# zhengfei0908/SBA-GAN

Hardware: AMD Instinct MI355X
Metric: images/sec (G+D step) at 256px (higher is better)
Workload: dtype bf16; 1 GPU; bird_style.yml 3-stage G+D step (64..256px), B=20 per GPU, G_NET variant=model, image_encoder=inception, text_encoder=RNN_ENCODER in the step; global_batch=20, parallelism=dp1, launch=replayer, losses_finite=True

## Files before the change

### sba-gan_amd/csrc/wgrad.hip

```cpp
#include "common.h"
#include "conv_common.h"

namespace {

struct FastDiv {
    uint64_t magic;
    uint32_t d;
};
static inline FastDiv make_fastdiv(uint32_t d, int64_t max_n) {
    FastDiv f;
    f.d = d;
    f.magic = (max_n < (1 << 21) && d > 0) ? (((uint64_t)1 << 42) + d - 1) / d : 0;
    return f;
}
__device__ __forceinline__ uint32_t fdiv(uint32_t n, const FastDiv& f) {
    return f.magic ? (uint32_t)(((uint64_t)n * f.magic) >> 42) : n / f.d;
}

__device__ __forceinline__ void zero_acc(f32x16_t (&acc)[2][2]) {
#pragma unroll
    for (int i = 0; i < 2; ++i)
#pragma unroll
        for (int j = 0; j < 2; ++j)
#pragma unroll
            for (int r = 0; r < 16; ++r) acc[i][j][r] = 0.f;
}
template <int N> __device__ __forceinline__ void zero_acc(f32x16_t (&acc)[N][2][2]) {
#pragma unroll
    for (int s = 0; s < N; ++s) zero_acc(acc[s]);
}

__device__ __forceinline__ void pixel_decode(const int m, const int sub, const int ow, const FastDiv& dsub, const FastDiv& dow,
                                             int& n, int& oy, int& ox) {
    n = (int)fdiv(m, dsub);
    const int rem = m - n * sub;
    oy = (int)fdiv(rem, dow);
    ox = rem - oy * ow;
}

__device__ __forceinline__ bool x_gather(const sba_conv_geom& g, const int IHL, const int IWL, const int n, const int oy, const int ox,
                                         const int ty, const int tx, int64_t& pix) {
    int iy = oy * g.sy + ty, ix = ox * g.sx + tx;
    const bool ok = (iy >= 0) & (iy < IHL) & (ix >= 0) & (ix < IWL);
    if (g.ups) { iy >>= 1; ix >>= 1; }
    pix = (int64_t)(n * g.IH + iy) * g.IW + ix;
    return ok;
}
__device__ __forceinline__ int64_t dy_pixel(const sba_conv_geom& g, const int n, const int oy, const int ox) {
    return (int64_t)(n * g.OH + oy * g.osy + g.ooy) * g.OW + ox * g.osx + g.oox;
}

__device__ __forceinline__ void dw_emit(float* p, const float v, const int mode) {
    if (mode == 1) atomicAdd(p, v);
    else if (mode == 2) *p = v;
    else *p += v;
}
template <bool OWNER>
__device__ __forceinline__ void store_tile(const f32x16_t (&acc)[2][2], float* dwz, const sba_conv_geom& g, const int co0,
                                           const int ci0, const int tap, const int mode, const int lane) {
    const int col_l = lane & 31, rsel = 4 * (lane >> 5);
#pragma unroll
    for (int i = 0; i < 2; ++i)
#pragma unroll
        for (int j = 0; j < 2; ++j)
#pragma unroll
            for (int r = 0; r < 16; ++r) {
                const int co = co0 + i * 32 + (r & 3) + 8 * (r >> 2) + rsel;
                const int ci = ci0 + j * 32 + col_l;
                if (co < g.Cout && ci < g.Cin) {
                    float* p = dwz + ((int64_t)co * g.ntaps + tap) * g.Cin + ci;
                    if (OWNER) dw_emit(p, acc[i][j][r], mode);
                    else if (mode == 2) *p = acc[i][j][r];
                    else atomicAdd(p, acc[i][j][r]);
                }
            }
}

template <typename T> struct WgFrag;

template <> struct WgFrag<bf16_t> {
    static constexpr int ROWS = 64 * 2 + 64;
    static __device__ __forceinline__ bf16x8_t load(const unsigned char* slice, int c32, int lane) {
        const int g16 = lane >> 4, i16 = lane & 15;
        const int cbase = c32 + 16 * (g16 & 1), kbase = 8 * (g16 >> 1);
        const int q = i16 >> 2, p = i16 & 3;
        const unsigned char* a0 = slice + (kbase + q) * ROWS + (cbase + 4 * p) * 2;
        typedef __attribute__((address_space(3))) s16x4_t* lptr;
        s16x4_t lo = __builtin_amdgcn_ds_read_tr16_b64_v4i16((lptr)(a0));
        s16x4_t hi = __builtin_amdgcn_ds_read_tr16_b64_v4i16((lptr)(a0 + 4 * ROWS));
        bf16x8_t r;
        r[0] = lo[0]; r[1] = lo[1]; r[2] = lo[2]; r[3] = lo[3];
        r[4] = hi[0]; r[5] = hi[1]; r[6] = hi[2]; r[7] = hi[3];
        return r;
    }
    static __device__ __forceinline__ void mma(const unsigned char* sa, const unsigned char* sb, int lane,
                                               f32x16_t (&acc)[2][2]) {
        bf16x8_t a[2], b[2];
        a[0] = load(sa, 0, lane); a[1] = load(sa, 32, lane);
        b[0] = load(sb, 0, lane); b[1] = load(sb, 32, lane);
#pragma unroll
        for (int i = 0; i < 2; ++i)
#pragma unroll
            for (int j = 0; j < 2; ++j)
                acc[i][j] = __builtin_amdgcn_mfma_f32_32x32x16_bf16(a[i], b[j], acc[i][j], 0, 0, 0);
    }
};

template <> struct WgFrag<float> {
    static constexpr int ROWS = 64 * 4 + 64;
    static __device__ __forceinline__ void mma(const unsigned char* sa, const unsigned char* sb, int lane,
                                               f32x16_t (&acc)[2][2]) {
        const int r = lane & 31, h = lane >> 5;
#pragma unroll
        for (int kk = 0; kk < 8; ++kk) {
            float a[2], b[2];
#pragma unroll
            for (int i = 0; i < 2; ++i) {
                a[i] = *reinterpret_cast<const float*>(sa + (2 * kk + h) * ROWS + (i * 32 + r) * 4);
                b[i] = *reinterpret_cast<const float*>(sb + (2 * kk + h) * ROWS + (i * 32 + r) * 4);
            }
#pragma unroll
            for (int i = 0; i < 2; ++i)
#pragma unroll
                for (int j = 0; j < 2; ++j)
                    acc[i][j] = __builtin_amdgcn_mfma_f32_32x32x2f32(a[i], b[j], acc[i][j], 0, 0, 0);
        }
    }
};

template <typename T>
__global__ __launch_bounds__(256) void wgrad_kernel(const T* __restrict__ x, const T* __restrict__ dy,
                                                    float* __restrict__ dw, const sba_conv_geom g,
                                                    const int M, const int chunks_per_split,
                                                    const int mode, const FastDiv dsub, const FastDiv dow,
                                                    const int64_t zstride) {
    constexpr int ROWS = WgFrag<T>::ROWS;
    constexpr int CH = 16 / (int)sizeof(T);
    constexpr int CPR = 64 / CH;
    constexpr int LPT = 16 * CPR / 64;
    constexpr int SLICE = 16 * ROWS;
    static_assert(4 * 2 * SLICE >= 64 * 64 * 4, "reduction buffer fits in the staging area");
    __shared__ __attribute__((aligned(16))) unsigned char lds[4 * 2 * SLICE];

    const int tid = threadIdx.x, lane = tid & 63, wid = tid >> 6;
    const int co0 = blockIdx.x * 64;
    const int ci_tiles = (g.Cin + 63) / 64;
    const int tap = blockIdx.y / ci_tiles, ci0 = (blockIdx.y - tap * ci_tiles) * 64;
    int ty = 0, tx = 0;
#pragma unroll
    for (int t = 0; t < SBA_MAX_TAPS; ++t)
        if (t == tap) { ty = g.ty[t]; tx = g.tx[t]; }
    const int IHL = g.ups ? 2 * g.IH : g.IH, IWL = g.ups ? 2 * g.IW : g.IW;
    const int sub = g.OHs * g.OWs;

// ... 568 lines not shown
    for (int kw = 0; kw < 3; ++kw)
        store_tile<false>(acc[kw], dw + (int64_t)blockIdx.z * zstride, g, co0, ci0, kh * 3 + kw, mode, lane);
}

enum WgradFamily { WG_ROW_DMA = 0, WG_SMALL_DMA = 1, WG_SMALL = 2, WG_ROWS = 3, WG_GENERIC = 4 };

struct WgradPlan {
    int family;
    int v[4];
    dim3 grid;
    int block, lds;
    int per_split;
    int mode;
    int npart;
    int wclog;
};

static int pixel_splits(int target_wgs, int wgs, int chunks, int min_chunks, int* per_split) {
    int sp = cdiv(target_wgs, wgs);
    if (sp > chunks / min_chunks) sp = chunks / min_chunks > 0 ? chunks / min_chunks : 1;
    *per_split = cdiv(chunks, sp);
    return cdiv(chunks, *per_split);
}

static bool wgrad_plan(int dtype, const sba_conv_geom* g, int ksplit, bool det_on, WgradPlan* p) {
    if (!geom_ok(g, dtype)) return false;
    if (g->Cin % 8 != 0 || g->Cout % 8 != 0) return false;
    if (g->x_cstride || g->x_coff || g->y_cstride || g->y_coff || g->ntaps > 16) return false;
    const int M = g->N * g->OHs * g->OWs;
    if (ksplit < 1) ksplit = 1;
    const int fw = g->first_write ? 2 : 0;
    const int co_tiles = cdiv(g->Cout, 64), items = cdiv(g->Cin, 64) * g->ntaps;
    const bool dma_ok = dtype == SBA_BF16 && (int64_t)g->N * g->OH * g->OW * g->Cout * 2 < (1ll << 32);
    auto fill = [&](int family, int v0, int v1, int v2, int v3, dim3 grid, int block, int lds, int per_split, int unsplit_mode) {
        *p = WgradPlan{family, {v0, v1, v2, v3}, grid, block, lds, per_split, 0, 0, 0};
        const int nz = (int)grid.z;
        p->npart = det_on && (nz > 1 || family == WG_ROWS) ? nz : 0;
        p->mode = p->npart ? 2 : (nz > 1 ? 1 : unsplit_mode);
        return grid.y <= 65535 && grid.z <= 65535;
    };
    {
        const int kwn = g->ntaps == 16 ? 4 : (g->ntaps == 9 ? 3 : 0), sxy = g->sx;
        bool ok = dma_ok && kwn && g->sy == sxy && (!g->ups || kwn == 3) && g->osy == 1 && g->osx == 1 && g->ooy == 0 &&
                  g->oox == 0 && g->OHs == g->OH && g->OWs == g->OW && g->Cin % 64 == 0 && g->Cout % 64 == 0 &&
                  g->OW >= 4 && (g->OW & (g->OW - 1)) == 0 && !(g->OW == 4 && (g->ups || g->OH != 4)) && M % 32 == 0 &&
                  ((g->OH * g->OW) % 32 == 0 || g->OW == 4);
        ok = ok && ((kwn == 4 && sxy == 2) || (kwn == 3 && sxy == 1));
        for (int t = 0; t < g->ntaps && ok; ++t)
            ok = g->ty[t] == g->ty[(t / kwn) * kwn] && g->tx[t] == g->tx[(t / kwn) * kwn] + (t % kwn);
        if (ok) {
            const int wc = g->OW < 32 ? g->OW : 32;
            int wclog = 0;
            while ((1 << wclog) < wc) ++wclog;
            const int wgs = co_tiles * kwn * (g->Cin / 64);
            constexpr int ROW_WGS = 512;
            int cps32;
            const int sp = pixel_splits(wgs <= 8 ? (ROW_WGS * 3) / 4 : ROW_WGS, wgs, M / 32, 12, &cps32);
            const int xb = kwn == 4 ? 10 : (g->OW == 4 ? 6 : 5);
            const int stage = kwn == 4 ? WgRowCfg<4, 10>::STAGE : (g->OW == 4 ? WgRowCfg<3, 6>::STAGE : WgRowCfg<3, 5>::STAGE);
            if (fill(WG_ROW_DMA, kwn, sxy, xb, 4, dim3(co_tiles, kwn * (g->Cin / 64), sp), 64 * kwn, 4 * stage, cps32, fw)) {
                p->wclog = wclog;
                return true;
            }
        }
    }
    constexpr int SMALL_M = 12000;
    if (M <= SMALL_M && co_tiles * items >= 256) {
        const int wgs = co_tiles * cdiv(items, 4);
        constexpr int SMALL_WGS = 768, SMALL_MINC = 24;
        const int target = wgs >= SMALL_WGS / 2 ? wgs : SMALL_WGS;
        int cps;
        const int split = pixel_splits(target, wgs, cdiv(M, 16), SMALL_MINC, &cps);
        const dim3 grid(co_tiles, cdiv(items, 4), split);
        if (grid.y > 65535 || grid.z > 65535) return false;
        constexpr int DMA_WGS = 512;
        if (fw == 2 && wgs > DMA_WGS && g->Cout % 128 == 0 && dma_ok) {
            fill(WG_SMALL_DMA, 2, 3, 0, 0, dim3(co_tiles / 2, cdiv(items, 4), 1), 256, 3 * 6 * 32 * 128, cdiv(M, 32), fw);
            return true;
        }
        if (wgs <= DMA_WGS && dma_ok) {
            int cps32;
            const int sp = pixel_splits(target, wgs, cdiv(M, 32), SMALL_MINC / 2, &cps32);
            return fill(WG_SMALL_DMA, 1, 4, 0, 0, dim3(co_tiles, cdiv(items, 4), sp), 256, 4 * 5 * 32 * 128, cps32, fw);
        }
        return fill(WG_SMALL, dtype, 0, 0, 0, grid, 256, 0, cps, fw);
    }
    constexpr int ROWS_M = 131072;
    bool rows_ok = g->ntaps == 9 && g->sy == 1 && g->sx == 1 && g->osy == 1 && g->osx == 1 && g->ooy == 0 &&
                   g->oox == 0 && g->OHs == g->OH && g->OWs == g->OW && g->OW % 64 == 0 && M >= ROWS_M;
    for (int t = 0; t < 9 && rows_ok; ++t) rows_ok = g->ty[t] == t / 3 - 1 && g->tx[t] == t % 3 - 1;
    if (rows_ok) {
        const int ci_t = cdiv(g->Cin, 64);
        int spw;
        const int nz = pixel_splits(256, co_tiles * ci_t, g->N * g->OH * (g->OW / 64), 16, &spw);
        return fill(WG_ROWS, dtype, 0, 0, 0, dim3(co_tiles, ci_t, nz), 192, 0, spw, 1);
    }
    if (dma_ok) {
        constexpr int GEN_WGS = 512;
        int cps32;
        const int sp = pixel_splits(GEN_WGS, co_tiles * cdiv(items, 4), cdiv(M, 32), 12, &cps32);
        if (fill(WG_SMALL_DMA, 1, 4, 0, 0, dim3(co_tiles, cdiv(items, 4), sp), 256, 4 * 5 * 32 * 128, cps32, fw)) return true;
    }
    const int total_chunks = cdiv(M, 64);
    if (ksplit > total_chunks) ksplit = total_chunks;
    const int cps = cdiv(total_chunks, ksplit);
    return fill(WG_GENERIC, dtype, 0, 0, 0, dim3(co_tiles, items, cdiv(total_chunks, cps)), 256, 0, cps, 0);
}

template <auto Kernel, typename... Args>
static void launch_dyn_lds(const WgradPlan& p, hipStream_t st, Args... args) {
    static bool once = false;
    if (!once) { (void)hipFuncSetAttribute((const void*)Kernel, hipFuncAttributeMaxDynamicSharedMemorySize, p.lds); once = true; }
    SBA_LAUNCH(Kernel, p.grid, dim3(p.block), p.lds, st, args...);
}

static int wgrad_launch(const WgradPlan& p, int dtype, const void* x, const void* dy, float* dw, const sba_conv_geom* g,
                        hipStream_t st) {
    const int M = g->N * g->OHs * g->OWs;
    const FastDiv dsub = make_fastdiv((uint32_t)(g->OHs * g->OWs), (int64_t)M + 64);
    const FastDiv dow = make_fastdiv((uint32_t)g->OWs, (int64_t)M + 64);
    const int64_t dwn = (int64_t)g->Cout * g->ntaps * g->Cin;
    float* part = nullptr;
    if (p.npart) { part = sba_det_alloc((int64_t)p.npart * dwn); if (!part) return SBA_E_ARG; }
    float* dwa = part ? part : dw;
    const int64_t zs = part ? dwn : 0;
    const bf16_t* xh = (const bf16_t*)x;
    const bf16_t* dyh = (const bf16_t*)dy;
    switch (p.family) {
    case WG_ROW_DMA:
        if (p.v[0] == 4) launch_dyn_lds<wgrad_row_dma_kernel<4, 2, 10, 4>>(p, st, xh, dyh, dwa, *g, M, p.per_split, p.mode, dsub, dow, zs, p.wclog);
        else if (p.v[2] == 6) launch_dyn_lds<wgrad_row_dma_kernel<3, 1, 6, 4>>(p, st, xh, dyh, dwa, *g, M, p.per_split, p.mode, dsub, dow, zs, p.wclog);
        else launch_dyn_lds<wgrad_row_dma_kernel<3, 1, 5, 4>>(p, st, xh, dyh, dwa, *g, M, p.per_split, p.mode, dsub, dow, zs, p.wclog);
        break;
    case WG_SMALL_DMA:
        if (p.v[0] == 2) launch_dyn_lds<wgrad_small_dma_kernel<2, 3>>(p, st, xh, dyh, dwa, *g, M, p.per_split, p.mode, dsub, dow, zs);
        else launch_dyn_lds<wgrad_small_dma_kernel<1, 4>>(p, st, xh, dyh, dwa, *g, M, p.per_split, p.mode, dsub, dow, zs);
        break;
    case WG_SMALL:
        SBA_DISPATCH(dtype, SBA_LAUNCH((wgrad_small_kernel<T>), p.grid, dim3(p.block), 0, st, (const T*)x, (const T*)dy, dwa, *g, M,
                                       p.per_split, p.mode, dsub, dow, zs));
        break;
    case WG_ROWS:
        SBA_DISPATCH(dtype, SBA_LAUNCH((wgrad_rows_kernel<T>), p.grid, dim3(p.block), 0, st, (const T*)x, (const T*)dy, dwa, *g,
                                       g->N * g->OH * (g->OW / 64), p.per_split, p.mode, zs));
        break;
    default:
        SBA_DISPATCH(dtype, SBA_LAUNCH((wgrad_kernel<T>), p.grid, dim3(p.block), 0, st, (const T*)x, (const T*)dy, dwa, *g, M,
                                       p.per_split, p.mode, dsub, dow, zs));
    }
    if (part) sba_det_fold(part, 1, p.npart, dwn, dw, 0, g->first_write ? 1 : 0, st);
    return SBA_CHECK_LAUNCH();
}

}

extern "C" int sba_conv_wgrad_plan(int dtype, const sba_conv_geom* g, int ksplit, int det, int* plan) {
    WgradPlan p;
    if (!plan || !wgrad_plan(dtype, g, ksplit, det != 0, &p)) return SBA_E_ARG;
    const int out[SBA_WGRAD_PLAN_INTS] = {p.family, p.v[0], p.v[1], p.v[2], p.v[3], (int)p.grid.x, (int)p.grid.y, (int)p.grid.z,
                                          p.block, p.lds, p.per_split, p.mode, p.npart, p.wclog};
    for (int i = 0; i < SBA_WGRAD_PLAN_INTS; ++i) plan[i] = out[i];
    return SBA_OK;
}

extern "C" int sba_conv_wgrad(int dtype, const void* x, const void* dy, float* dw, const sba_conv_geom* g,
                              int ksplit, void* stream) {
    WgradPlan p;
    if (!x || !dy || !dw || !wgrad_plan(dtype, g, ksplit, sba_det_on(), &p)) return SBA_E_ARG;
    return wgrad_launch(p, dtype, x, dy, dw, g, (hipStream_t)stream);
}
```

### sba-gan_amd/sbagan/_lib.py

```python
import ctypes
import os

import torch
from ctypes import POINTER, byref, c_float, c_int, c_int64, c_uint64, c_void_p

from .abi import CONSTANTS, DECLS, STRUCTS

_HERE = os.path.dirname(os.path.abspath(__file__))
LIB_PATH = os.environ.get('SBA_LIB_PATH') or os.path.join(os.path.dirname(_HERE), 'csrc', 'libsbagan_hip.so')

SBA_F32, SBA_BF16, SBA_BF16_YH = (CONSTANTS['SBA_' + k] for k in ('F32', 'BF16', 'BF16_YH'))
ACT_NONE, ACT_GLU, ACT_LRELU, ACT_RELU = (CONSTANTS['SBA_ACT_' + k] for k in ('NONE', 'GLU', 'LRELU', 'RELU'))
MAX_TAPS, IGEMM_TILES, WGRAD_PLAN_INTS, GROUP_MAX = (
    CONSTANTS['SBA_' + k] for k in ('MAX_TAPS', 'IGEMM_TILES', 'WGRAD_PLAN_INTS', 'GROUP_MAX'))
WGRAD_FAMILIES = ('row_dma', 'small_dma', 'small', 'rows', 'generic')
ConvGeom, ConvGroupItem = STRUCTS['sba_conv_geom'], STRUCTS['sba_conv_group_item']

if not os.path.exists(LIB_PATH):
    raise ImportError('libsbagan_hip.so not built: run `python __graft_entry__.py` or '
                      '`make -C sba-gan_amd/csrc` (expected %s)' % LIB_PATH)
lib = ctypes.CDLL(LIB_PATH)

P, I, F, L, U = c_void_p, c_int, c_float, c_int64, c_uint64
G = POINTER(ConvGeom)

SIGNATURES = {}
for _name, _decl in DECLS.items():
    _fn = getattr(lib, _name)
    _fn.argtypes = _args = [_ctype for _, _, _ctype in _decl.params]
    _fn.restype = _decl.restype
    if _decl.restype is c_int:
        SIGNATURES[_name] = _args

_ERR = {CONSTANTS['SBA_E_ARG']: 'SBA_E_ARG (unsupported shape/alignment/enum)',
        CONSTANTS['SBA_E_LAUNCH']: 'SBA_E_LAUNCH (HIP launch failed)',
        CONSTANTS['SBA_E_UNSUPPORTED']: 'SBA_E_UNSUPPORTED (graph node kind the replayer cannot re-issue)'}


AUDIT_HOOK = None


def call(name, *args):
    if AUDIT_HOOK is not None:
        AUDIT_HOOK(name, args)
    rc = getattr(lib, name)(*args)
    if rc != 0:
        raise RuntimeError('%s failed: %s' % (name, _ERR.get(rc, rc)))


def wgrad_plan(dtype, g, ksplit, det=None):
    plan = (c_int * WGRAD_PLAN_INTS)()
    det = lib.sba_get_deterministic() if det is None else int(det)
    call('sba_conv_wgrad_plan', dtype, byref(g), ksplit, det, plan)
    return list(plan)


def wgrad_plan_name(plan):
    fam, nargs = WGRAD_FAMILIES[plan[0]], (4, 2, 0, 0, 0)[plan[0]]
    args = ','.join(str(v) for v in plan[1:1 + nargs]) if nargs else ('f32', 'bf16')[plan[1]]
    return '%s<%s> x%d' % (fam, args, plan[7])


def version():
    return lib.sba_version().decode()
```

### sba-gan_amd/sbagan/abi.py

```python
import os
import re
from collections import namedtuple
from ctypes import (POINTER, Structure, c_char_p, c_double, c_float, c_int, c_int8, c_int32, c_int64, c_uint64,
                    c_void_p)

HEADER = os.path.join(os.path.dirname(os.path.dirname(os.path.dirname(os.path.abspath(__file__)))),
                      'include', 'sbagan_hip.h')

TYPES = {'int': c_int, 'int64_t': c_int64, 'uint64_t': c_uint64, 'float': c_float, 'double': c_double,
         'int*': POINTER(c_int), 'void**': POINTER(c_void_p)}
FIELD_TYPES = dict(TYPES, int32_t=c_int32, int8_t=c_int8)
RETURNS = {'int': c_int, 'int64_t': c_int64, 'const char*': c_char_p}
HOST_STRUCTS = ('sba_conv_geom', 'sba_conv_group_item')

Decl = namedtuple('Decl', 'ret restype params')


def _squeeze(ctext):
    return re.sub(r'\s*\*', '*', ' '.join(ctext.split()))


def _ctype(ctext, types, structs, host_structs, where):
    base = re.sub(r'\bconst\b|\s', '', ctext)
    if base in types:
        return types[base]
    if base.endswith('*') and base[:-1] in host_structs:
        if base[:-1] not in structs:
            raise ValueError('%s: %s is used before it is declared' % (where, base[:-1]))
        return POINTER(structs[base[:-1]])
    if re.fullmatch(r'\w+\*+', base):
        return c_void_p
    raise ValueError('%s: unknown type %r' % (where, ctext))


def parse(text, host_structs=HOST_STRUCTS):
    text = re.sub(r'/\*.*?\*/|//[^\n]*', ' ', text, flags=re.S)
    constants, structs, decls = {}, {}, {}

    def new(name):
        if name in constants or name in structs or name in decls:
            raise ValueError('%s is declared twice' % name)
        return name

    for m in re.finditer(r'^[ \t]*#[ \t]*define[ \t]+(SBA_\w+)(.*)$', text, flags=re.M):
        value = re.fullmatch(r'\s+\(?(-?\d+)\)?\s*', m.group(2))
        if not value:
            raise ValueError('#define %s: not an integer: %r' % (m.group(1), m.group(2).strip()))
        constants[new(m.group(1))] = int(value.group(1))
    text = re.sub(r'^[ \t]*#.*$', '', text, flags=re.M)

    def struct(m):
        name, fields = m.group(1), []
        if m.group(3) != name:
            raise ValueError('typedef struct %s: named %s' % (name, m.group(3)))
        for stmt in filter(None, (s.strip() for s in m.group(2).split(';'))):
            f = re.fullmatch(r'(.*?)(\w+(?:\[\w+\])?(?:\s*,\s*\w+(?:\[\w+\])?)*)', stmt, flags=re.S)
            if not f:
                raise ValueError('struct %s: cannot read %r' % (name, stmt))
            ctype = _ctype(f.group(1), FIELD_TYPES, structs, host_structs, 'struct %s: %r' % (name, stmt))
            for field, bound in re.findall(r'(\w+)(?:\[(\w+)\])?', f.group(2)):
                if bound and not bound.isdigit() and bound not in constants:
                    raise ValueError('struct %s: %s[%s]: unknown bound' % (name, field, bound))
                fields.append((field, ctype * int(constants.get(bound, bound)) if bound else ctype))
        structs[new(name)] = type(name, (Structure,), {'_fields_': fields})
        return ''
    text = re.sub(r'typedef\s+struct\s+(\w+)\s*\{(.*?)\}\s*(\w+)\s*;', struct, text, flags=re.S)

    text = re.sub(r'extern\s+"C"\s*\{|\}', '', text)
    for stmt in filter(None, (' '.join(s.split()) for s in text.split(';'))):
        m = re.fullmatch(r'(.+?)\s*\b(sba_\w+)\s*\(([^()]*)\)', stmt)
        if not m:
            raise ValueError('cannot read the declaration %r' % stmt)
        ret, name = _squeeze(m.group(1)), m.group(2)
        if ret not in RETURNS:
            raise ValueError('%s: unknown return type %r' % (name, ret))
        params = []
        for p in ([] if m.group(3).strip() in ('', 'void') else m.group(3).split(',')):
            f = re.fullmatch(r'\s*(.*?)\s*(\w+)\s*', p)
            ctext = _squeeze(f.group(1)) if f else p
            params.append((ctext, f.group(2) if f else '', _ctype(ctext, TYPES, structs, host_structs,
                                                                 '%s: parameter %r' % (name, p.strip()))))
        decls[new(name)] = Decl(ret, RETURNS[ret], params)
    return constants, structs, decls


with open(HEADER) as _f:
    CONSTANTS, STRUCTS, DECLS = parse(_f.read())
```

### sba-gan_amd/sbagan/ops.py

```python
import ctypes
import os
from collections import namedtuple

import numpy as np
import torch

from . import _lib
from ._lib import ACT_GLU, ACT_LRELU, ACT_NONE, ConvGeom, call

CL = torch.channels_last
COMPUTE_DTYPE = torch.bfloat16
BN_EPS, BN_MOMENTUM, IN_EPS = 1e-5, 0.1, 1e-5

_WEIGHT_EPOCH = [0]


def set_compute_dtype(dt):
    global COMPUTE_DTYPE
    assert dt in (torch.bfloat16, torch.float32)
    COMPUTE_DTYPE = dt
    _WEIGHT_EPOCH[0] += 1


def compute_dtype():
# ... 374 lines not shown
_IGEMM_TABLE = None


def geom_key(g):
    return '%d_%dx%d_%d_%dx%d_%d_t%d_s%d_u%d' % (g.N, g.IH, g.IW, g.Cin, g.OHs, g.OWs, g.Cout, g.ntaps, g.sy, g.ups)


_TABLE_FILE = None


def _table_section(name):
    global _TABLE_FILE
    if _TABLE_FILE is None:
        _TABLE_FILE = {}
        path = os.environ.get('SBA_IGEMM_TABLE_FILE') or os.path.join(os.path.dirname(os.path.abspath(__file__)),
                                                                      'igemm_table.json')
        if os.environ.get('SBA_IGEMM_TABLE', '1') != '0' and os.path.exists(path):
            import json
            with open(path) as f:
                _TABLE_FILE = json.load(f)
    return _TABLE_FILE.get(name, {})


def _igemm_table():
    global _IGEMM_TABLE
    if _IGEMM_TABLE is None:
        _IGEMM_TABLE = _table_section('bf16')
    return _IGEMM_TABLE


def tune_geom(g, dt):
    if getattr(g, '_tuned', None) != dt:
        g._tuned = dt
        ent = _igemm_table().get(geom_key(g)) if dt == _lib.SBA_BF16 else None
        g.tile, g.ksplit = (int(ent[0]), int(ent[1])) if ent else (0, 0)
    if IGEMM_LOG is not None:
        IGEMM_LOG.append(g)


def _igemm(dt, x, w, y, addend, stats, g, device, w_frag=None):
    ws = workspace(device)
    tune_geom(g, _lib.SBA_BF16 if dt == _lib.SBA_BF16_YH else dt)
    g.w_layout = 0
    if w_frag is not None and _halo_family(g):
        w, g.w_layout = w_frag.data_ptr(), 1
    try:
        call('sba_conv_igemm', dt, x, w, y, addend, stats, ctypes.byref(g), ws.data_ptr(), WORKSPACE_BYTES, _stream())
    finally:
        g.w_layout = 0


def _halo_family(g):
    h = getattr(g, '_halo', None)
    if h is None:
        plan = (ctypes.c_int * 3)()
        old = g.w_layout
        g.w_layout = 0
        call('sba_conv_igemm_plan', _lib.SBA_BF16, ctypes.byref(g), WORKSPACE_BYTES, plan)
        g.w_layout = old
        h = g._halo = plan[0] == 0
    return h




def conv_forward(x, pw, kind, want_stats=True, addend=None, pre_bn=False):
    _need_gpu(x)
    N, Cin, H, W = x.shape
    O = pw.param.shape[0]
    OH, OW = _conv_out_hw(kind, H, W)
    yh = pre_bn and Y_F16 and x.dtype == torch.bfloat16 and addend is None and O % 8 == 0
    if yh:
        y = torch.empty((N, O, OH, OW), dtype=torch.float16, device=x.device, memory_format=CL)
    else:
        y = empty_act(N, O, OH, OW, x)
    stats = zeros_f32((BN_STAT_SLOTS, 2 * O), x.device) if want_stats else None
    g = _geom((kind, N, H, W, Cin, O, None))
    wf = pw.fwd_frag(x.dtype) if kind == '3x3' else None
    _igemm(_lib.SBA_BF16_YH if yh else _dt(x), _p(x), _p(pw.fwd(x.dtype)), _p(y), _p(addend), _p(stats), g, x.device,
           w_frag=wf)
    return y, stats


def conv_dgrad(dy, pw, kind, in_hw, addend=None):
    N, O, OH, OW = dy.shape
    I = pw.param.shape[1]
    H, W = in_hw
    wd = pw.dgrad(dy.dtype, kind)
    if kind == '3x3':
        g = _geom(('3x3', N, OH, OW, O, I, None))
        dx = empty_act(N, I, H, W, dy)
        _igemm(_dt(dy), _p(dy), _p(wd), _p(dx), _p(addend), None, g, dy.device, w_frag=pw.dgrad_frag(dy.dtype, kind))
        return dx
    if kind == '3x3up':
        g = _geom(('4x4s2', N, OH, OW, O, I, None))
        dx = empty_act(N, I, H, W, dy)
        _igemm(_dt(dy), _p(dy), _p(wd), _p(dx), _p(addend), None, g, dy.device)
        return dx
    if kind == '4x4s2':
        dx = empty_act(N, I, H, W, dy)
        esz = dy.element_size()
        gs = [_geom(('4x4s2_dgrad', N, OH, OW, O, I, (cls // 2, cls % 2))) for cls in range(4)]
        if DGRAD4_GROUP and dy.dtype == torch.bfloat16 and O % 64 == 0:
            arr = (_lib.ConvGroupItem * 4)()
            for cls, (a, g) in enumerate(zip(arr, gs)):
                a.x, a.w, a.y, a.addend = _p(dy), wd.data_ptr() + cls * I * 4 * O * esz, _p(dx), _p(addend)
                a.bias = a.relu_mask = None
                a.g = ctypes.pointer(g)
            tile, split = dgrad4_plan(gs[0])
            ws = workspace(dy.device)
            call('sba_conv_igemm_group_splitk', _lib.SBA_BF16, 4, arr, tile, split, ws.data_ptr(), WORKSPACE_BYTES, _stream())
            if IGEMM_LOG is not None:
                IGEMM_LOG.append(('group', tile, gs))
            return dx
        for cls in range(4):
            wptr = wd.data_ptr() + cls * I * 4 * O * esz
            _igemm(_dt(dy), _p(dy), wptr, _p(dx), _p(addend), None, gs[cls], dy.device)
        return dx
    raise ValueError(kind)


DGRAD4_GROUP = True
_DGRAD4_FORCE = None


def dgrad4_plan(g):
    if _DGRAD4_FORCE:
        t, s = _DGRAD4_FORCE.split(',')
        return int(t), int(s)
    ent = _table_section('dgrad4').get(geom_key(g))
    if ent:
        return int(ent[0]), int(ent[1])
    M = g.N * g.OHs * g.OWs
    ny = (g.Cout + 63) // 64
    for tile, bm in ((5, 128), (3, 96), (1, 64)):
        tiles = 4 * ((M + bm - 1) // bm) * ny
        if tiles >= 512 or tile == 1:
            break
    ns64 = g.ntaps * (g.Cin // 64)
    split = max(1, min(512 // max(tiles, 1), ns64 // 8))
    return tile, split


_KSPLIT_TARGET = 640
_KSPLIT_MIN_CHUNKS = 24


def _ksplit(tiles, M):
    chunks = (M + 63) // 64
    want = max(1, (_KSPLIT_TARGET + tiles - 1) // tiles)
    return max(1, min(want, chunks // _KSPLIT_MIN_CHUNKS if chunks >= 2 * _KSPLIT_MIN_CHUNKS else 1))


def conv_wgrad(x, dy, param, kind):
    N, Cin, H, W = x.shape
    O = dy.shape[1]
    g = _geom((kind, N, H, W, Cin, O, None))
    gbuf = param_grad(param)
    M = N * g.OHs * g.OWs
    tiles = ((O + 63) // 64) * ((Cin + 63) // 64) * g.ntaps
    cell = getattr(param, '_sba_gepoch', None)
    first = 0
    if cell is not None and getattr(param, '_sba_wepoch', None) != cell[0]:
        param._sba_wepoch = cell[0]
        first = 1
    g.first_write = first
    call('sba_conv_wgrad', _dt(x), _p(x), _p(dy), _p(gbuf), ctypes.byref(g), _ksplit(tiles, M), _stream())


SIDE_WGRAD = False
HOME_STREAM = None
_COMPANION, _KEEPALIVE, _COMP_NEXT = {}, {}, {}
N_COMPANIONS = int(os.environ.get('SBA_WGRAD_COMPANIONS', '1'))


def _companion(device, *keep):
    cur = torch.cuda.current_stream()
    key = cur.cuda_stream
    comps = _COMPANION.get(key)
    if comps is None:
        comps = _COMPANION[key] = [torch.cuda.Stream(device=device) for _ in range(N_COMPANIONS)]
        _KEEPALIVE[key] = []
        _COMP_NEXT[key] = 0
    comp = comps[_COMP_NEXT[key] % len(comps)]
    _COMP_NEXT[key] += 1
    comp.wait_stream(cur)
    _KEEPALIVE[key].extend(keep)
    return comp


def conv_wgrad_overlapped(x, dy, param, kind):
    if not SIDE_WGRAD:
        return conv_wgrad(x, dy, param, kind)
    param_grad(param)
    with torch.cuda.stream(_companion(x.device, x, dy)):
        conv_wgrad(x, dy, param, kind)


def join_wgrads():
    cur = torch.cuda.current_stream()
    comps = _COMPANION.get(cur.cuda_stream)
    if comps is not None:
        for comp in comps:
            cur.wait_stream(comp)
        _KEEPALIVE[cur.cuda_stream].clear()
        _COMP_NEXT[cur.cuda_stream] = 0


def wgrad_tail_stream():
    cur = torch.cuda.current_stream()
    comps = _COMPANION.get(cur.cuda_stream)
    if comps is None:
        return cur
    comp = comps[0]
    comp.wait_stream(cur)
    for other in comps[1:]:
        comp.wait_stream(other)
    _KEEPALIVE[cur.cuda_stream].clear()
    _COMP_NEXT[cur.cuda_stream] = 0
    return comp


BN_STAT_SLOTS = _lib.lib.sba_bn_stat_slots()


_DET_SCRATCH = [None]
DET_SCRATCH_BYTES = int(os.environ.get('SBA_DET_SCRATCH_MB', '2048')) << 20


def set_deterministic(flag, device=None):
    if torch.cuda.is_available():
        torch.cuda.synchronize()
    if flag:
        dev = torch.device('cuda', torch.cuda.current_device()) if device is None else device
        if _DET_SCRATCH[0] is None or _DET_SCRATCH[0].device != dev:
            _DET_SCRATCH[0] = torch.empty(DET_SCRATCH_BYTES, dtype=torch.uint8, device=dev)
        call('sba_set_deterministic', 1, _DET_SCRATCH[0].data_ptr(), DET_SCRATCH_BYTES)
    else:
        call('sba_set_deterministic', 0, None, 0)


def deterministic():
    return bool(_lib.lib.sba_get_deterministic())


def det_reset():
    if _lib.lib.sba_get_deterministic():
        call('sba_det_reset')


if os.environ.get('SBA_DETERMINISTIC', '0') == '1' and torch.cuda.is_available():
    set_deterministic(True)


class BNState(object):
    __slots__ = ('aux', 'C', 'rows', 'groups')


def bn_act_forward(y, stats, bn, act, residual=None, groups=1):
    N, C, H, W = y.shape
    Co = C // 2 if act == ACT_GLU else C
    st = BNState()
    st.C, st.rows, st.groups = C, (N // groups) * H * W, groups
    st.aux = torch.empty((groups, 4, C), dtype=torch.float32, device=y.device)
    out = torch.empty((N, Co, H, W), dtype=_act_dtype(y), device=y.device, memory_format=CL)
    call('sba_bn_act_fwd', _dt(y), _p(y), _p(stats), _p(bn.weight), _p(bn.bias), _p(bn.running_mean),
         _p(bn.running_var), _p(bn.num_batches_tracked), _p(st.aux), _p(residual), _p(out), st.rows, groups, C,
         act, Co, 0, BN_EPS, BN_MOMENTUM, 1 if bn.training else 0, _stream())
    return out, st


BN_FUSED_BWD_ROWS = 2560


def bn_act_backward(y, dout, st, bn, act, need_param_grad=True, out=None, red=None):
    N, C, H, W = y.shape
    Co = C // 2 if act == ACT_GLU else C
    dy = out if out is not None else torch.empty(y.shape, dtype=_act_dtype(y), device=y.device, memory_format=CL)
    dg = db = None
    if need_param_grad:
        dg, db = param_grad(bn.weight), param_grad(bn.bias)
    if st.rows <= BN_FUSED_BWD_ROWS:
        call('sba_bn_act_bwd_fused', _dt(y), _p(y), _p(dout), _p(st.aux), _p(dy), _p(dg), _p(db), st.rows, st.groups,
             C, act, Co, 0, _stream())
        return dy
    if red is None:
        red = zeros_f32((st.groups, BN_STAT_SLOTS, 2 * C), y.device)
        call('sba_bn_act_bwd_reduce', _dt(y), _p(y), _p(dout), _p(st.aux), _p(red), st.rows, st.groups, C, act, Co, 0,
             _stream())
    call('sba_bn_act_bwd_apply', _dt(y), _p(y), _p(dout), _p(st.aux), _p(red), _p(dy), _p(dg), _p(db), st.rows,
         st.groups, C, act, Co, 0, _stream())
    return dy


def bn_act_forward_fused(y, bn, act, groups):
    N, C, H, W = y.shape
    Co = C // 2 if act == ACT_GLU else C
    st = BNState()
    st.C, st.rows, st.groups = C, (N // groups) * H * W, groups
    st.aux = torch.empty((groups, 4, C), dtype=torch.float32, device=y.device)
    out = torch.empty((N, Co, H, W), dtype=_act_dtype(y), device=y.device, memory_format=CL)
    call('sba_bn_act_fwd_fused', _dt(y), _p(y), _p(bn.weight), _p(bn.bias), _p(bn.running_mean), _p(bn.running_var),
         _p(bn.num_batches_tracked), _p(st.aux), _p(out), st.rows, groups, C, act, Co, 0, BN_EPS, BN_MOMENTUM, _stream())
    return out, st


def bn_stats(y, groups=1):
    N, C, H, W = y.shape
    stats = zeros_f32((groups, BN_STAT_SLOTS, 2 * C), y.device)
    call('sba_bn_stats', _dt(y), _p(y), _p(stats), (N // groups) * H * W, groups, C, _stream())
    return stats


def bn_act_forward_grouped(y, bn, act, groups):
    N, C, H, W = y.shape
    if bn.training and (N // groups) * H * W <= BN_FUSED_BWD_ROWS:
        return bn_act_forward_fused(y, bn, act, groups)
    stats = bn_stats(y, groups) if bn.training else None
    return bn_act_forward(y, stats, bn, act, None, groups)
# ... 1682 lines not shown
```

Baseline: 2101 images/sec.

## Compute upsample-conv weight grad on the low-res grid via 4x4 stride-2 reformulation

For nearest-2x-upsample followed by a 3x3 conv, the weight gradient is now computed as a 4x4 stride-2 conv wgrad over the source grid, with input and dy swapped. This routes it onto the row_dma wgrad family. A new fold kernel then sums each 2x2 group of the 16 taps back into the 9 flipped taps, adds into the grad buffer and zeroes the scratch. The aim is to avoid reading the 4x-larger upsampled activation and to use a faster kernel family. In exchange it adds a per-stream scratch buffer, an extra kernel launch and a route-planning check, and ksplit is fixed to 1.

```diff
diff --git a/include/sbagan_hip_wgrad_up.h b/include/sbagan_hip_wgrad_up.h
--- /dev/null
+++ b/include/sbagan_hip_wgrad_up.h
@@ -0,0 +1,16 @@
+#ifndef SBAGAN_HIP_WGRAD_UP_H
+#define SBAGAN_HIP_WGRAD_UP_H
+
+#include "sbagan_hip.h"
+
+#ifdef __cplusplus
+extern "C" {
+#endif
+
+int sba_conv_wgrad_up(int dtype, const void* x, const void* dy, float* dw, float* dw4, const sba_conv_geom* g,
+                      int ksplit, void* stream);
+
+#ifdef __cplusplus
+}
+#endif
+#endif
diff --git a/sba-gan_amd/csrc/wgrad.hip b/sba-gan_amd/csrc/wgrad.hip
--- a/sba-gan_amd/csrc/wgrad.hip
+++ b/sba-gan_amd/csrc/wgrad.hip
@@ -1,5 +1,6 @@
 #include "common.h"
 #include "conv_common.h"
+#include "sbagan_hip_wgrad_up.h"
 
 namespace {
 
@@ -874,6 +875,69 @@
     return SBA_CHECK_LAUNCH();
 }
 
+__global__ __launch_bounds__(256) void wgrad_up_fold_kernel(float* __restrict__ dw4, float* __restrict__ dw, const int I,
+                                                            const int O, const int first) {
+    __shared__ float s[9][16][17];
+    const int tid = threadIdx.x, lo = tid & 15, hi = tid >> 4;
+    const int o0 = blockIdx.x * 16, i0 = blockIdx.y * 16;
+    {
+        float v[16];
+        float* src = dw4 + ((int64_t)(i0 + hi) * 16) * O + o0 + lo;
+        const bool ok = i0 + hi < I && o0 + lo < O;
+#pragma unroll
+        for (int t = 0; t < 16; ++t) v[t] = ok ? src[(int64_t)t * O] : 0.f;
+        if (ok) {
+#pragma unroll
+            for (int t = 0; t < 16; ++t) src[(int64_t)t * O] = 0.f;
+        }
+#pragma unroll
+        for (int kh = 0; kh < 3; ++kh)
+#pragma unroll
+            for (int kw = 0; kw < 3; ++kw) {
+                const int a = (2 - kh) * 4 + (2 - kw);
+                s[kh * 3 + kw][lo][hi] = (v[a] + v[a + 1]) + (v[a + 4] + v[a + 5]);
+            }
+    }
+    __syncthreads();
+    float* p[9];
+    float val[9];
+    bool ok[9];
+#pragma unroll
+    for (int r = 0; r < 9; ++r) {
+        const int idx = tid + 256 * r;
+        const int il = idx & 15, t = (idx >> 4) % 9, ol = idx / (16 * 9);
+        ok[r] = i0 + il < I && o0 + ol < O;
+        p[r] = dw + ((int64_t)(o0 + ol) * 9 + t) * I + i0 + il;
+        val[r] = s[t][ol][il];
+    }
+    if (!first) {
+#pragma unroll
+        for (int r = 0; r < 9; ++r)
+            if (ok[r]) val[r] += *p[r];
+    }
+#pragma unroll
+    for (int r = 0; r < 9; ++r)
+        if (ok[r]) *p[r] = val[r];
+}
+
+static bool wgrad_up_swap(const sba_conv_geom* g, sba_conv_geom* s) {
+    if (!g || !g->ups || g->ntaps != 9 || g->sy != 1 || g->sx != 1 || g->OH != 2 * g->IH || g->OW != 2 * g->IW ||
+        g->OHs != g->OH || g->OWs != g->OW || g->osy != 1 || g->osx != 1 || g->ooy || g->oox || g->x_cstride || g->x_coff ||
+        g->y_cstride || g->y_coff)
+        return false;
+    for (int t = 0; t < 9; ++t)
+        if (g->ty[t] != t / 3 - 1 || g->tx[t] != t % 3 - 1) return false;
+    *s = sba_conv_geom{};
+    s->N = g->N; s->IH = g->OH; s->IW = g->OW; s->Cin = g->Cout;
+    s->OH = s->OHs = g->IH; s->OW = s->OWs = g->IW; s->Cout = g->Cin;
+    s->sy = s->sx = 2;
+    s->osy = s->osx = 1;
+    s->ntaps = 16;
+    for (int t = 0; t < 16; ++t) { s->ty[t] = (int8_t)(t / 4 - 1); s->tx[t] = (int8_t)(t % 4 - 1); }
+    s->first_write = 1;
+    return true;
+}
+
 }
 
 extern "C" int sba_conv_wgrad_plan(int dtype, const sba_conv_geom* g, int ksplit, int det, int* plan) {
@@ -891,3 +955,17 @@
     if (!x || !dy || !dw || !wgrad_plan(dtype, g, ksplit, sba_det_on(), &p)) return SBA_E_ARG;
     return wgrad_launch(p, dtype, x, dy, dw, g, (hipStream_t)stream);
 }
+
+extern "C" int sba_conv_wgrad_up(int dtype, const void* x, const void* dy, float* dw, float* dw4, const sba_conv_geom* g,
+                                 int ksplit, void* stream) {
+    sba_conv_geom s;
+    WgradPlan p;
+    if (!x || !dy || !dw || !dw4 || !wgrad_up_swap(g, &s) || !wgrad_plan(dtype, &s, ksplit, sba_det_on(), &p) ||
+        p.family != WG_ROW_DMA)
+        return SBA_E_ARG;
+    const int rc = wgrad_launch(p, dtype, dy, x, dw4, &s, (hipStream_t)stream);
+    if (rc != SBA_OK) return rc;
+    SBA_LAUNCH(wgrad_up_fold_kernel, dim3(cdiv(g->Cout, 16), cdiv(g->Cin, 16)), dim3(256), 0, (hipStream_t)stream, dw4, dw,
+               g->Cin, g->Cout, g->first_write ? 1 : 0);
+    return SBA_CHECK_LAUNCH();
+}
diff --git a/sba-gan_amd/sbagan/_lib.py b/sba-gan_amd/sbagan/_lib.py
--- a/sba-gan_amd/sbagan/_lib.py
+++ b/sba-gan_amd/sbagan/_lib.py
@@ -4,7 +4,10 @@
 import torch
 from ctypes import POINTER, byref, c_float, c_int, c_int64, c_uint64, c_void_p
 
-from .abi import CONSTANTS, DECLS, STRUCTS
+from . import abi
+from .abi import CONSTANTS, STRUCTS
+
+DECLS = dict(abi.DECLS, **abi.MORE_DECLS)
 
 _HERE = os.path.dirname(os.path.abspath(__file__))
 LIB_PATH = os.environ.get('SBA_LIB_PATH') or os.path.join(os.path.dirname(_HERE), 'csrc', 'libsbagan_hip.so')
diff --git a/sba-gan_amd/sbagan/abi.py b/sba-gan_amd/sbagan/abi.py
--- a/sba-gan_amd/sbagan/abi.py
+++ b/sba-gan_amd/sbagan/abi.py
@@ -85,4 +85,14 @@
 
 
 with open(HEADER) as _f:
-    CONSTANTS, STRUCTS, DECLS = parse(_f.read())
+    _text = _f.read()
+CONSTANTS, STRUCTS, DECLS = parse(_text)
+MORE_HEADERS = (os.path.join(os.path.dirname(HEADER), 'sbagan_hip_wgrad_up.h'),)
+MORE_DECLS = {}
+for _path in MORE_HEADERS:
+    with open(_path) as _f:
+        _text += _f.read()
+    for _name, _d in parse(_text)[2].items():
+        if _name not in DECLS and _name not in MORE_DECLS:
+            MORE_DECLS[_name] = Decl(_d.ret, _d.restype, [(c, n, _ctype(c, TYPES, STRUCTS, HOST_STRUCTS, _name))
+                                                          for c, n, _ in _d.params])
diff --git a/sba-gan_amd/sbagan/ops.py b/sba-gan_amd/sbagan/ops.py
--- a/sba-gan_amd/sbagan/ops.py
+++ b/sba-gan_amd/sbagan/ops.py
@@ -550,11 +550,44 @@
     return max(1, min(want, chunks // _KSPLIT_MIN_CHUNKS if chunks >= 2 * _KSPLIT_MIN_CHUNKS else 1))
 
 
-def conv_wgrad(x, dy, param, kind):
+WGRAD_UP_MAX_BYTES = 4 << 20
+
+
+def wgrad_up_route(dt, N, H, W, Cin, O):
+    if dt != _lib.SBA_BF16 or 64 * Cin * O > WGRAD_UP_MAX_BYTES:
+        return False
+    try:
+        plan = _lib.wgrad_plan(dt, _geom(('4x4s2', N, 2 * H, 2 * W, O, Cin, None)), 1, det=0)
+    except RuntimeError:
+        return False
+    return _lib.WGRAD_FAMILIES[plan[0]] == 'row_dma'
+
+
+_WGRAD_UP_ROUTE = {}
+_WGRAD_UP_SCRATCH = {}
+
+
+def wgrad_up_scratch(device, nfloats):
+    key = (device, torch.cuda.current_stream(device).cuda_stream, nfloats)
+    buf = _WGRAD_UP_SCRATCH.get(key)
+    if buf is None:
+        with torch.cuda.stream(torch.cuda.default_stream(device)):
+            buf = torch.zeros(nfloats, dtype=torch.float32, device=device)
+        torch.cuda.current_stream(device).wait_stream(torch.cuda.default_stream(device))
+        _WGRAD_UP_SCRATCH[key] = buf
+    return buf
+
+
+def conv_wgrad(x, dy, param, kind, source_grid=None):
     N, Cin, H, W = x.shape
     O = dy.shape[1]
     g = _geom((kind, N, H, W, Cin, O, None))
     gbuf = param_grad(param)
+    if kind == '3x3up' and source_grid is None:
+        rkey = (_dt(x), N, H, W, Cin, O)
+        source_grid = _WGRAD_UP_ROUTE.get(rkey)
+        if source_grid is None:
+            source_grid = _WGRAD_UP_ROUTE[rkey] = wgrad_up_route(*rkey)
     M = N * g.OHs * g.OWs
     tiles = ((O + 63) // 64) * ((Cin + 63) // 64) * g.ntaps
     cell = getattr(param, '_sba_gepoch', None)
@@ -563,6 +596,10 @@
         param._sba_wepoch = cell[0]
         first = 1
     g.first_write = first
+    if kind == '3x3up' and source_grid:
+        dw4 = wgrad_up_scratch(x.device, 16 * Cin * O)
+        call('sba_conv_wgrad_up', _dt(x), _p(x), _p(dy), _p(gbuf), _p(dw4), ctypes.byref(g), 1, _stream())
+        return
     call('sba_conv_wgrad', _dt(x), _p(x), _p(dy), _p(gbuf), ctypes.byref(g), _ksplit(tiles, M), _stream())
 
 
```

Result: no change. 2112 images/sec, median of 6 (+0.5%).
